# Hxyz-123/GoMatching

Hardware: AMD Instinct MI355X
Metric: frames/sec (whole node), 1280x720 clip, 100 queries/frame (higher is better)
Workload: dtype f32 (f16x3 split MFMA: 22-bit significand products, fp32 accumulate; parity tests at fp32 tolerances)

## Files before the change

### gomatching_amd/csrc/bneck_fused.hip

```cpp
#include "common.h"

namespace {

constexpr int CH = 32;
constexpr int FRAG = 1024;
constexpr int BM = 128;
constexpr int XT_ROW = 36;

struct BnArgs {
    const float* A;
    const unsigned char* img;
    const float* R;
    const float* sc1;
    const float* sh1;
    float* X;
    float* Y1;
    int* flag;
    int lda, ldr, ldx, ldy, M, chunks;
};

template <int K1, int MP>
struct Cfg {
    static constexpr int W3_FRAGS = (K1 / 16) * 2;
    static constexpr int W1_FRAGS = (MP / 32) * 2 * 2;
    static constexpr int STAGE_FRAGS = W3_FRAGS + W1_FRAGS + 1;
    static constexpr int STAGE_BYTES = STAGE_FRAGS * FRAG;
    static constexpr int XTR = (K1 == 64 && MP == 64) ? 32 : 16;
    static constexpr int XT_BYTES = XTR * XT_ROW * 4;
    static constexpr int LDS_BYTES = 2 * STAGE_BYTES + 4 * XT_BYTES;
};

template <int K1, int MP, int OCC>
__global__ __launch_bounds__(256, OCC) void bneck_kernel(const BnArgs p) {
    using C = Cfg<K1, MP>;
    extern __shared__ __attribute__((aligned(16))) unsigned char smem[];
    const int tid = threadIdx.x, lane = tid & 63;
    const int wave = __builtin_amdgcn_readfirstlane(tid >> 6);
    const int fr = lane & 31, fh = lane >> 5;
    const long m = (long)blockIdx.x * BM + wave * 32 + fr;
    const long row = m < p.M ? m : p.M - 1;
    const unsigned lane16 = lane * 16;

    const __amdgpu_buffer_rsrc_t rs_img = gom_buffer_rsrc(p.img, p.chunks * C::STAGE_BYTES);
    auto dma_stage = [&](int c, int slot) {
        for (int f = wave; f < C::STAGE_FRAGS; f += 4)
            gom_dma_fragment(rs_img, lane16, (unsigned)c * C::STAGE_BYTES + f * FRAG, smem + slot * C::STAGE_BYTES + f * FRAG);
    };

    float amax = 0.f, chk = 0.f;
    half8 xf[2][K1 / 16];
    long crow[4];
#pragma unroll
    for (int i = 0; i < 4; ++i) {
        const long mm = (long)blockIdx.x * BM + wave * 32 + (lane >> 3) + 8 * i;
        crow[i] = mm < p.M ? mm : p.M - 1;
    }
    const int cpc = (lane & 7) * 4;
    float* xt = reinterpret_cast<float*>(smem + 2 * C::STAGE_BYTES + wave * C::XT_BYTES);
    constexpr int XTR = C::XTR, PASSES = 32 / XTR, RPP = XTR / 8;
    f32x4 rv[4];
    {
        const float* xr = p.A + (size_t)row * p.lda + fh * 8;
        f32x4 ra[K1 / 8];
#pragma unroll
        for (int s = 0; s < K1 / 16; ++s) {
            ra[2 * s] = *reinterpret_cast<const f32x4*>(xr + 16 * s);
            ra[2 * s + 1] = *reinterpret_cast<const f32x4*>(xr + 16 * s + 4);
        }
#pragma unroll
        for (int i = 0; i < 4; ++i) rv[i] = *reinterpret_cast<const f32x4*>(p.R + (size_t)crow[i] * p.ldr + cpc);
        __builtin_amdgcn_sched_barrier(0);
        dma_stage(0, 0);
        __builtin_amdgcn_sched_barrier(0);
#pragma unroll
        for (int s = 0; s < K1 / 16; ++s) {
#pragma unroll
            for (int e = 0; e < 4; ++e) amax = fmaxf(amax, fmaxf(fabsf(ra[2 * s][e]), fabsf(ra[2 * s + 1][e])));
            gom_split8_f16(ra[2 * s], ra[2 * s + 1], xf[0][s], xf[1][s]);
        }
        asm volatile("" : "+v"(amax));
    }

    f32x16 acc2[MP / 32];
#pragma unroll
    for (int t = 0; t < MP / 32; ++t)
#pragma unroll
        for (int g = 0; g < 16; ++g) acc2[t][g] = 0.f;

    asm volatile("s_waitcnt vmcnt(0)" ::: "memory");
    __syncthreads();

    for (int c = 0; c < p.chunks; ++c) {
        const int st = c & 1;
        const unsigned char* base = smem + st * C::STAGE_BYTES + lane16;
        const float* aux = reinterpret_cast<const float*>(smem + st * C::STAGE_BYTES + (C::W3_FRAGS + C::W1_FRAGS) * FRAG);
        if (c + 1 < p.chunks) dma_stage(c + 1, st ^ 1);
        f32x4 rn[4];
#pragma unroll
        for (int q = 0; q < 4; ++q) {
            rn[q] = f32x4{0.f, 0.f, 0.f, 0.f};
            if (c + 1 < p.chunks) rn[q] = *reinterpret_cast<const f32x4*>(p.R + (size_t)crow[q] * p.ldr + CH * (c + 1) + cpc);
        }
        f32x4 ra4[4];
#pragma unroll
        for (int hp = 0; hp < PASSES; ++hp) {
#pragma unroll
            for (int i = 0; i < RPP; ++i) *reinterpret_cast<f32x4*>(xt + ((lane >> 3) + 8 * i) * XT_ROW + cpc) = rv[RPP * hp + i];
            __builtin_amdgcn_wave_barrier();
            if (PASSES == 1 || (fr >> 4) == hp) {
#pragma unroll
                for (int q = 0; q < 4; ++q) ra4[q] = *reinterpret_cast<const f32x4*>(xt + (fr & (XTR - 1)) * XT_ROW + 8 * q + 4 * fh);
            }
            __builtin_amdgcn_wave_barrier();
        }
        f32x16 acc1;
#pragma unroll
        for (int g = 0; g < 16; ++g) acc1[g] = 0.f;
#pragma unroll
        for (int s = 0; s < K1 / 16; ++s) {
            const half8 w_hi = *reinterpret_cast<const half8*>(base + (2 * s) * FRAG);
            const half8 w_lo = *reinterpret_cast<const half8*>(base + (2 * s + 1) * FRAG);
            acc1 = __builtin_amdgcn_mfma_f32_32x32x16_f16(w_hi, xf[1][s], acc1, 0, 0, 0);
            acc1 = __builtin_amdgcn_mfma_f32_32x32x16_f16(w_lo, xf[0][s], acc1, 0, 0, 0);
            acc1 = __builtin_amdgcn_mfma_f32_32x32x16_f16(w_hi, xf[0][s], acc1, 0, 0, 0);
        }
        half8 hf[2][2];
        f32x4 vx[4];
#pragma unroll
        for (int u = 0; u < 2; ++u) {
            f32x4 v[2];
#pragma unroll
            for (int qq = 0; qq < 2; ++qq) {
                const int q = 2 * u + qq;
                const f32x4 sc = *reinterpret_cast<const f32x4*>(aux + 8 * q + 4 * fh);
                const f32x4 sh = *reinterpret_cast<const f32x4*>(aux + CH + 8 * q + 4 * fh);
#pragma unroll
                for (int e = 0; e < 4; ++e) {
                    const float t = acc1[4 * q + e] * sc[e] + sh[e] + ra4[q][e];
                    chk = fmaf(t, 0.f, chk);
                    v[qq][e] = fmaxf(t, 0.f);
                    amax = fmaxf(amax, v[qq][e]);
                }
                vx[q] = v[qq];
            }
            gom_split8_f16(v[0], v[1], hf[0][u], hf[1][u]);
        }
#pragma unroll
        for (int hp = 0; hp < PASSES; ++hp) {
            if (PASSES == 1 || (fr >> 4) == hp) {
#pragma unroll
                for (int q = 0; q < 4; ++q) *reinterpret_cast<f32x4*>(xt + (fr & (XTR - 1)) * XT_ROW + 8 * q + 4 * fh) = vx[q];
            }
            __builtin_amdgcn_wave_barrier();
#pragma unroll
            for (int i = 0; i < RPP; ++i) {
                const f32x4 o = *reinterpret_cast<const f32x4*>(xt + ((lane >> 3) + 8 * i) * XT_ROW + cpc);
                *reinterpret_cast<f32x4*>(p.X + (size_t)crow[RPP * hp + i] * p.ldx + CH * c + cpc) = o;
            }
            __builtin_amdgcn_wave_barrier();
        }
#pragma unroll
        for (int t = 0; t < MP / 32; ++t)
#pragma unroll
            for (int u = 0; u < 2; ++u) {
                const half8 w_hi = *reinterpret_cast<const half8*>(base + (C::W3_FRAGS + (t * 2 + u) * 2) * FRAG);
                const half8 w_lo = *reinterpret_cast<const half8*>(base + (C::W3_FRAGS + (t * 2 + u) * 2 + 1) * FRAG);
                acc2[t] = __builtin_amdgcn_mfma_f32_32x32x16_f16(w_hi, hf[1][u], acc2[t], 0, 0, 0);
                acc2[t] = __builtin_amdgcn_mfma_f32_32x32x16_f16(w_lo, hf[0][u], acc2[t], 0, 0, 0);
                acc2[t] = __builtin_amdgcn_mfma_f32_32x32x16_f16(w_hi, hf[0][u], acc2[t], 0, 0, 0);
            }
#pragma unroll
        for (int q = 0; q < 4; ++q) rv[q] = rn[q];
        asm volatile("s_waitcnt vmcnt(4)" ::: "memory");
        __syncthreads();
    }

    float* yrow = p.Y1 + (size_t)row * p.ldy + 4 * fh;
#pragma unroll
    for (int t = 0; t < MP / 32; ++t)
#pragma unroll
        for (int q = 0; q < 4; ++q) {
            const int col = 32 * t + 8 * q + 4 * fh;
            const f32x4 sc = *reinterpret_cast<const f32x4*>(p.sc1 + col);
            const f32x4 sh = *reinterpret_cast<const f32x4*>(p.sh1 + col);
            f32x4 o;
#pragma unroll
            for (int e = 0; e < 4; ++e) {
                const float tv = acc2[t][4 * q + e] * sc[e] + sh[e];
                chk = fmaf(tv, 0.f, chk);
                o[e] = fmaxf(tv, 0.f);
            }
            *reinterpret_cast<f32x4*>(yrow + 32 * t + 8 * q) = o;
        }
    if ((!(amax <= 65504.f) || !(chk == 0.f)) && p.flag) atomicOr(p.flag, 1);
}

__global__ __launch_bounds__(256) void bneck_image_kernel(const unsigned short* __restrict__ p3, long ps3, int ld3,
                                                          const float* __restrict__ inv3, const float* __restrict__ scale3,
                                                          const float* __restrict__ shift3, const unsigned short* __restrict__ p1,
                                                          long ps1, int ld1, int k1, int c4, int mp, unsigned short* __restrict__ img) {
    const int w3f = (k1 / 16) * 2, w1f = (mp / 32) * 4, sf = w3f + w1f + 1;
    const long i = (long)blockIdx.x * 256 + threadIdx.x;
    const long total = (long)(c4 / CH) * sf * 512;
    if (i >= total) return;
    const int e = (int)(i % 512), f = (int)((i / 512) % sf), c = (int)(i / (512L * sf));
    const int l = e >> 3, j = e & 7, r = l & 31, h = l >> 5;
    if (f < w3f) {
        const int s = f >> 1, pl = f & 1;
        img[i] = p3[pl * ps3 + (size_t)(CH * c + r) * ld3 + 16 * s + 8 * h + j];
    } else if (f < w3f + w1f) {
        const int id = f - w3f, t = id >> 2, u = (id >> 1) & 1, pl = id & 1;
        img[i] = p1[pl * ps1 + (size_t)(32 * t + r) * ld1 + CH * c + 16 * u + 8 * (j >> 2) + 4 * h + (j & 3)];
    } else {
        const int fi = e >> 1;
        float v = 0.f;
        if (fi < CH) v = inv3[CH * c + fi] * (scale3 ? scale3[CH * c + fi] : 1.f);
        else if (fi < 2 * CH) v = shift3 ? shift3[CH * c + fi - CH] : 0.f;
        const unsigned bits = __builtin_bit_cast(unsigned, v);
        img[i] = (unsigned short)((e & 1) ? (bits >> 16) : (bits & 0xffffu));
    }
}

template <int K1, int MP, int OCC>
int launch(const BnArgs& a, hipStream_t s) {
    using C = Cfg<K1, MP>;
    auto kern = bneck_kernel<K1, MP, OCC>;
    if (C::LDS_BYTES > 65536) {
        hipError_t e = hipFuncSetAttribute((const void*)kern, hipFuncAttributeMaxDynamicSharedMemorySize, C::LDS_BYTES);
        if (e != hipSuccess) return GOM_ERR_HIP_BASE + (int)e;
    }
    hipLaunchKernelGGL(kern, dim3((unsigned)cdiv(a.M, BM)), dim3(256), C::LDS_BYTES, s, a);
    return gom_launch_status();
}

bool served(int k1, int c4, int mp) {
    if (c4 != 4 * k1) return false;
    return (k1 == 64 && (mp == 64 || mp == 128)) || (k1 == 128 && (mp == 128 || mp == 256));
}

}

extern "C" long gom_bneck_image_bytes(int k1, int c4, int mp) {
    if (!served(k1, c4, mp)) return -1;
    return (long)(c4 / CH) * ((k1 / 16) * 2 + (mp / 32) * 4 + 1) * FRAG;
}

extern "C" int gom_bneck_image(const void* w3_planes, long w3_plane_stride, int ld3, const float* w3_inv_scale, const float* scale3,
                               const float* shift3, const void* w1_planes, long w1_plane_stride, int ld1, int k1, int c4, int mp,
                               void* image, long image_bytes, void* stream) {
    GOM_CHECK_ARG(w3_planes && w3_inv_scale && w1_planes && image && served(k1, c4, mp) && ld3 >= k1 && ld1 >= c4);
    GOM_CHECK_ARG(image_bytes >= gom_bneck_image_bytes(k1, c4, mp));
    const long total = (long)(c4 / CH) * ((k1 / 16) * 2 + (mp / 32) * 4 + 1) * 512;
    hipLaunchKernelGGL(bneck_image_kernel, dim3((unsigned)cdiv(total, 256)), dim3(256), 0, (hipStream_t)stream,
                       (const unsigned short*)w3_planes, w3_plane_stride, ld3, w3_inv_scale, scale3, shift3,
                       (const unsigned short*)w1_planes, w1_plane_stride, ld1, k1, c4, mp, (unsigned short*)image);
    return gom_launch_status();
}

extern "C" int gom_bneck_f32(const float* A, int lda, const void* image, const float* R, int ldr, const float* scale1,
                             const float* shift1, float* X, int ldx, float* Y1, int ldy, int M, int k1, int c4, int mp, int* flag,
                             void* stream) {
    GOM_CHECK_ARG(A && image && R && scale1 && shift1 && X && Y1 && M >= 0 && served(k1, c4, mp));
    GOM_CHECK_ARG(lda >= k1 && ldr >= c4 && ldx >= c4 && ldy >= mp && (lda % 4) == 0 && (ldr % 4) == 0 && (ldx % 4) == 0 && (ldy % 4) == 0);
    GOM_CHECK_ARG(((uintptr_t)A % 16) == 0 && ((uintptr_t)R % 16) == 0 && ((uintptr_t)X % 16) == 0 && ((uintptr_t)Y1 % 16) == 0 &&
                  ((uintptr_t)image % 16) == 0 && ((uintptr_t)scale1 % 16) == 0 && ((uintptr_t)shift1 % 16) == 0);
    if (M == 0) return GOM_OK;
    BnArgs a{};
    a.A = A; a.img = (const unsigned char*)image; a.R = R; a.sc1 = scale1; a.sh1 = shift1; a.X = X; a.Y1 = Y1; a.flag = flag;
    a.lda = lda; a.ldr = ldr; a.ldx = ldx; a.ldy = ldy; a.M = M; a.chunks = c4 / CH;
    hipStream_t s = (hipStream_t)stream;
    if (k1 == 64 && mp == 64) return launch<64, 64, 3>(a, s);
    if (k1 == 64 && mp == 128) return launch<64, 128, 2>(a, s);
    if (k1 == 128 && mp == 128) return launch<128, 128, 2>(a, s);
    return launch<128, 256, 1>(a, s);
}
```

### gomatching_amd/lib.py

```python
import ctypes
import os
from ctypes import c_int, c_long, c_float, c_void_p

HERE = os.path.dirname(os.path.abspath(__file__))
LIB_PATH = os.environ.get("GOM_LIB_PATH") or os.path.join(HERE, "libgomatching_hip.so")

GOM_OK = 0
_ERR = {1: "GOM_ERR_INVALID_ARG (violated precondition)", 2: "GOM_ERR_UNSUPPORTED"}

P = c_void_p
I = c_int
L = c_long
F = c_float

SIGNATURES = {
    "gom_abi_version": (I, []),
    "gom_built_for_arch": (ctypes.c_char_p, []),
    "gom_ms_deform_attn_forward": (I, [P, P, P, P, P, P, I, I, I, I, I, I, I, P]),
    "gom_ms_deform_attn_forward_any": (I, [I, P, P, P, P, P, P, I, I, I, I, I, I, I, P]),
    "gom_ms_deform_attn_backward": (I, [I, P, P, P, P, P, P, P, P, P, I, I, I, I, I, I, I, P]),
    "gom_ms_deform_attn_forward_strided": (I, [P, L, I, P, P, P, P, P, I, I, P]),
    "gom_msda_set_lane_distributed": (I, [I]),
    "gom_msda_fused_forward": (I, [P, I, P, P, L, I, P, P, P, I, I, P]),
    "gom_msda_fused_forward_encoder": (I, [P, I, P, P, L, I, P, P, P, I, I, I, I, I, I, P]),
    "gom_msda_set_window": (I, [I]),
    "gom_msda_window_count_fallbacks": (I, [P]),
    "gom_msda_prepare": (I, [P, I, P, I, P, P, P, L, P]),
    "gom_gemm_f32": (I, [P, P, P, I, P, I, P, P, P, I, I, P, I, I, I, I, P]),
    "gom_gemm_splitk_workspace_bytes": (L, [I, I, I]),
    "gom_gemm_f32_splitk": (I, [P, P, I, P, I, P, P, P, I, I, P, I, I, I, I, P, L, P]),
    "gom_conv2d_nhwc_f32": (I, [P, P, P, P, P, I, P, I, I, I, I, I, I, I, I, I, P]),
    "gom_split_bf16x3": (I, [P, I, I, I, P, I, P]),
    "gom_gemm_f32_bf16x6": (I, [P, P, I, P, L, I, P, P, P, I, I, I, P, I, I, I, I, P]),
    "gom_conv2d_nhwc_f32_bf16x6": (I, [P, P, L, I, P, P, P, I, P, I, I, I, I, I, I, I, I, I, P]),
    "gom_gemm_small_f32": (I, [P, P, I, P, I, P, P, P, I, I, P, I, I, I, I, P]),
    "gom_conv_bf16x6_splits": (I, [I, I, I]),
    "gom_conv2d_nhwc_f32_bf16x6_splitk": (I, [P, P, L, I, P, P, P, I, P, I, I, I, I, I, I, I, I, I, P, L, I, P]),
    "gom_split_f16x2": (I, [P, I, I, I, P, I, P, P]),
    "gom_gemm_f32_f16x3": (I, [P, P, I, P, L, I, P, P, P, P, I, I, I, P, I, I, I, I, P, P]),
    "gom_gemm_f32_f16x3_rp": (I, [P, P, I, P, L, I, P, P, P, P, I, I, I, I, P, I, I, I, I, P, P]),
    "gom_conv2d_nhwc_f32_f16x3": (I, [P, P, L, I, P, P, P, P, I, P, I, I, I, I, I, I, I, I, I, P, L, I, P, P]),
    "gom_conv3x3_patch_supported": (I, [I, I]),
    "gom_conv3x3_patch_image_bytes": (L, [I, I]),
    "gom_conv3x3_patch_image": (I, [P, L, I, I, I, P, L, P]),
    "gom_conv3x3_patch_f32_f16x3": (I, [P, P, P, P, P, I, P, I, I, I, I, I, P, P]),
    "gom_bneck_image_bytes": (L, [I, I, I]),
    "gom_bneck_image": (I, [P, L, I, P, P, P, P, L, I, I, I, I, P, L, P]),
    "gom_bneck_f32": (I, [P, I, P, P, I, P, P, P, I, P, I, I, I, I, I, P, P]),
    "gom_bneck2_image_bytes": (L, [I, I, I]),
    "gom_bneck2_image": (I, [P, L, I, P, P, P, P, L, I, I, I, I, P, L, P]),
    "gom_bneck2_f32": (I, [P, I, P, P, I, P, P, P, I, P, I, I, I, I, I, P, P]),
    "gom_dec_attn_image_bytes": (L, [I, I]),
    "gom_dec_attn_image": (I, [P, L, I, P, P, P, L, I, P, P, P, P, I, P, L, P]),
    "gom_dec_attn_f32": (I, [P, I, P, I, P, F, P, I, I, I, I, I, P, P]),
    "gom_dec_attn_raw_image_bytes": (L, []),
    "gom_dec_attn_raw_image": (I, [P, L, I, P, P, P, L, P]),
    "gom_dec_attn_raw_f32": (I, [P, I, P, F, P, I, P, I, P, I, I, I, I, P, P]),
    "gom_dec_attn2_image_bytes": (L, [I, I]),
    "gom_dec_attn2_image": (I, [P, L, I, P, P, P, L, I, P, P, P, P, I, P, L, P]),
    "gom_dec_attn2_f32": (I, [P, I, P, I, P, F, P, I, I, I, I, I, P, P]),
    "gom_dec_attn2_raw_image_bytes": (L, []),
    "gom_dec_attn2_raw_image": (I, [P, L, I, P, P, P, L, P]),
    "gom_dec_attn2_raw_f32": (I, [P, I, P, F, P, I, P, I, P, I, I, I, I, P, P]),
    "gom_dec_inter_heads_f32": (I, [P, I, P, P, I, I, I, I, P, P]),
    "gom_proj_ln_image_bytes": (L, [I, I]),
    "gom_proj_ln_image": (I, [P, L, I, I, I, P, L, P]),
    "gom_proj_ln_f32": (I, [P, I, P, P, P, P, I, P, P, F, P, I, I, P, P]),
    "gom_proj_ln_dot_f32": (I, [P, I, P, P, P, P, P, F, P, F, P, I, P, P]),
    "gom_gemm_k256_image_bytes": (L, [I, I]),
    "gom_gemm_k256_image": (I, [P, L, I, P, P, I, I, P, L, P]),
    "gom_gemm_k256_f32": (I, [P, P, I, P, P, I, I, I, P, I, I, I, I, I, P, P]),
    "gom_gemm_k256_rp_f32": (I, [P, P, I, P, P, I, I, I, I, P, I, I, I, I, I, P, P]),
    "gom_gemm_k256_set_lines": (None, [I]),
    "gom_gemm_k256_set_interleave": (None, [I]),
    "gom_stem_conv_pool_f32": (I, [P, P, L, I, P, P, P, P, I, I, I, P, P]),
    "gom_ffn_fused_image_bytes": (L, [I, I]),
    "gom_ffn_fused_image": (I, [P, L, I, P, P, P, L, I, I, I, P, L, P]),
    "gom_ffn_set_half_tail": (I, [I]),
    "gom_ffn_set_stream_cus": (I, [I]),
    "gom_ffn_fused_ln_f32": (I, [P, I, P, P, P, P, P, F, P, I, I, I, I, P, P]),
    "gom_ffn_fused_image_acc_order": (I, [P, L, I, P, P, P, L, I, I, I, P, L, P]),
# ... 114 lines not shown
```

### gomatching_amd/modeling/backbone.py

```python
import torch

from .. import ops

_STAGES = (("res2", 3, 1), ("res3", 4, 2), ("res4", 6, 2), ("res5", 3, 2))


def _fold_bn(sd, name, device, eps=1e-5):
    scale = sd[name + ".norm.weight"] * (sd[name + ".norm.running_var"] + eps).rsqrt()
    shift = sd[name + ".norm.bias"] - sd[name + ".norm.running_mean"] * scale
    return scale.float().contiguous().to(device), shift.float().contiguous().to(device)


def _ohwi(w, device, pad_cin_to=None):
    w = w.float().permute(0, 2, 3, 1)
    if pad_cin_to is not None and w.shape[-1] < pad_cin_to:
        w = torch.cat([w, w.new_zeros(w.shape[:-1] + (pad_cin_to - w.shape[-1],))], -1)
    return w.contiguous().to(device)


class ResNet50:
    out_features = ("res3", "res4", "res5")
    strides = {"res3": 8, "res4": 16, "res5": 32}
    channels = {"res3": 512, "res4": 1024, "res5": 2048}

    def __init__(self, sd, device, prefix="backbone.0.backbone."):
        self.device = device
        self.convs = {}

        def add(name, pad_cin_to=None):
            w = ops.prep_conv_weight(_ohwi(sd[prefix + name + ".weight"], device, pad_cin_to))
            sc, sh = _fold_bn(sd, prefix + name, device)
            self.convs[name] = (w, sc, sh)

        add("stem.conv1", pad_cin_to=4)
        self.blocks = []
        for stage, nblk, first_stride in _STAGES:
            for i in range(nblk):
                p = "%s.%d." % (stage, i)
                has_sc = (prefix + p + "shortcut.weight") in sd
                if has_sc:
                    add(p + "shortcut")
                for c in ("conv1", "conv2", "conv3"):
                    add(p + c)
                self.blocks.append((stage, p, first_stride if i == 0 else 1, has_sc, i == nblk - 1))
        self.fused = {}
        for (_, p, _, _, _), (_, pn, _, _, _) in zip(self.blocks[:-1], self.blocks[1:]):
            w3, sc3, sh3 = self.convs[p + "conv3"]
            w1, sc1, sh1 = self.convs[pn + "conv1"]
            if ops.BneckFused.serves(w3, w1):
                self.fused[p] = ops.BneckFused(w3, sc3, sh3, w1, sc1, sh1)

    def _conv(self, x, name, stride=1, pad=0, relu=False, R=None):
        w, sc, sh = self.convs[name]
        return ops.conv2d_nhwc(x, w, scale=sc, shift=sh, R=R, relu=relu, stride=stride, pad=pad)

    def forward(self, x_nhwc4):
        w, sc, sh = self.convs["stem.conv1"]
        if ops.stem_pool_serves(w):
            x = ops.stem_conv_pool(x_nhwc4.contiguous(), w, scale=sc, shift=sh)
        else:
            x = self._conv(x_nhwc4, "stem.conv1", stride=2, pad=3, relu=True)
            x = ops.maxpool3x3s2(x)
        outs = {}
        y1 = None
        for stage, p, s, has_sc, last in self.blocks:
            sc = self._conv(x, p + "shortcut", stride=s) if has_sc else x
            y = y1 if y1 is not None else self._conv(x, p + "conv1", relu=True)
            y = self._conv(y, p + "conv2", stride=s, pad=1, relu=True)
            blk = self.fused.get(p)
            if blk is not None:
                x, y1 = ops.bneck_fused(y, blk, sc)
            else:
                x, y1 = self._conv(y, p + "conv3", relu=True, R=sc), None
            if last:
                outs[stage] = x
        return {k: outs[k] for k in self.out_features}
```

### gomatching_amd/ops.py

```python
import contextlib
import ctypes
import math

import numpy as np
import torch

from . import lib as _lib_mod
from .lib import check

_f32 = torch.float32


def _L():
    return _lib_mod.load()


_gemm_profile = None


_profile_scope = ""


@contextlib.contextmanager
def profile_scope(name):
# ... 503 lines not shown
    if prof is not None:
        e1.record()
        prof.append((e0, e1, 2.0 * M * 256 * 256, (12.0 if R is not None else 8.0) * M * 256 + blk.image.numel(),
                     "projln:%dx256x256" % M, _profile_scope))
    return out


PROPOSAL_DOT = _switch("PROPOSAL_DOT")


def proj_ln_dot(x, blk, w, b):
    assert x.dim() == 2 and x.stride(1) == 1 and x.shape[1] == 256 and x.dtype == _f32
    _chk_f32(w)
    assert w.numel() == 256
    M = x.shape[0]
    out = torch.empty((M,), dtype=_f32, device=x.device)
    prof = _gemm_profile if (_gemm_profile is not None and M > 0) else None
    if prof is not None:
        e0, e1 = torch.cuda.Event(enable_timing=True), torch.cuda.Event(enable_timing=True)
        e0.record()
    check(_L().gom_proj_ln_dot_f32(_p(x), x.stride(0) if M > 1 else 256, _p(blk.image), _p(blk.W.inv_scale), _p(blk.bias),
                                   _p(blk.gamma), _p(blk.beta), blk.eps, _p(w), float(b), _p(out), M, _p(range_flag(x.device)),
                                   _stream()), "gom_proj_ln_dot_f32")
    if prof is not None:
        e1.record()
        prof.append((e0, e1, 2.0 * M * 256 * 257, 4.0 * M * 257 + blk.image.numel(), "projdot:%dx256x257" % M, _profile_scope))
    return out


BNECK_FUSED = _switch("BNECK_FUSED")


BNECK2 = _switch("BNECK2")


class BneckFused:

    def __init__(self, w3, scale3, shift3, w1, scale1, shift1):
        assert isinstance(w3, SplitWeight) and isinstance(w1, SplitWeight) and w3.kind == "f16x3" and w1.kind == "f16x3"
        self.k1, self.c4, self.mp = w3.K, w3.N, w1.N
        assert w1.K == self.c4
        _chk_f32(scale3, shift3, scale1, shift1)
        p3, p1 = w3.planes, w1.planes
        self.v2 = BneckFused._wide(self.k1, self.c4, self.mp)
        if self.v2:
            nbytes = _L().gom_bneck2_image_bytes(self.k1, self.c4, self.mp)
            self.image = torch.empty((nbytes,), dtype=torch.uint8, device=p3.device)
            check(_L().gom_bneck2_image(_p(p3), p3.stride(0), p3.stride(1), _p(w3.inv_scale), _p(scale3), _p(shift3), _p(p1), p1.stride(0),
                                        p1.stride(1), self.k1, self.c4, self.mp, _p(self.image), nbytes, _stream()), "gom_bneck2_image")
            self.sc1 = (scale1 * w1.inv_scale).contiguous()
            self.sh1 = shift1.contiguous()
            return
        nbytes = _L().gom_bneck_image_bytes(self.k1, self.c4, self.mp)
        if nbytes < 0:
            raise _lib_mod.GomError("fused bottleneck kernel does not serve %d -> %d -> %d" % (self.k1, self.c4, self.mp))
        self.image = torch.empty((nbytes,), dtype=torch.uint8, device=p3.device)
        check(_L().gom_bneck_image(_p(p3), p3.stride(0), p3.stride(1), _p(w3.inv_scale), _p(scale3), _p(shift3), _p(p1), p1.stride(0),
                                   p1.stride(1), self.k1, self.c4, self.mp, _p(self.image), nbytes, _stream()), "gom_bneck_image")
        self.sc1 = (scale1 * w1.inv_scale).contiguous()
        self.sh1 = shift1.contiguous()

    @staticmethod
    def _wide(k1, c4, mp):
        return bool(BNECK2) and _L().gom_bneck2_image_bytes(k1, c4, mp) > 0

    @staticmethod
    def serves(w3, w1):
        return (BNECK_FUSED and GEMM_MODE == "f16x3" and isinstance(w3, SplitWeight) and isinstance(w1, SplitWeight)
                and w3.kind == "f16x3" and w1.kind == "f16x3" and w1.K == w3.N
                and (BneckFused._wide(w3.K, w3.N, w1.N) or _L().gom_bneck_image_bytes(w3.K, w3.N, w1.N) > 0))


def bneck_fused(a, blk, R):
    _chk_f32(a, R)
    B, H, W, k1 = a.shape
    assert k1 == blk.k1 and tuple(R.shape) == (B, H, W, blk.c4) and a.is_contiguous() and R.is_contiguous()
    M = B * H * W
    X = torch.empty((B, H, W, blk.c4), dtype=_f32, device=a.device)
    Y1 = torch.empty((B, H, W, blk.mp), dtype=_f32, device=a.device)
    prof = _gemm_profile if (_gemm_profile is not None and M > 0) else None
    if prof is not None:
        e0, e1 = torch.cuda.Event(enable_timing=True), torch.cuda.Event(enable_timing=True)
        e0.record()
    fn = _L().gom_bneck2_f32 if blk.v2 else _L().gom_bneck_f32
    check(fn(_p(a), k1, _p(blk.image), _p(R), blk.c4, _p(blk.sc1), _p(blk.sh1), _p(X), blk.c4, _p(Y1), blk.mp, M,
             blk.k1, blk.c4, blk.mp, _p(range_flag(a.device)), _stream()), "gom_bneck2_f32" if blk.v2 else "gom_bneck_f32")
    if prof is not None:
        e1.record()
        prof.append((e0, e1, 2.0 * M * blk.c4 * (blk.k1 + blk.mp), 4.0 * M * (blk.k1 + 2 * blk.c4 + blk.mp) + blk.image.numel(),
                     "bneck:%dx%dx%dx%d" % (M, blk.k1, blk.c4, blk.mp), _profile_scope))
    return X, Y1


DEC_ATTN = _switch("DEC_ATTN")
DEC_ATTN_INTRA = _switch("DEC_ATTN_INTRA")
DEC_ATTN_INTER = _switch("DEC_ATTN_INTER")


class DecAttnBlock:

    def __init__(self, in_w, in_b, out_w, out_b, gamma, beta, inter, eps=1e-5, raw=None, form=None):
        self.form = form if form is not None else (2 if DEC_ATTN2 else 1)
        assert tuple(in_w.shape) == (768, 256) and tuple(out_w.shape) == (256, 256)
        nbytes = _L().gom_dec_attn_image_bytes(256, 8)
        if nbytes < 0:
            raise _lib_mod.GomError("decoder attention kernel serves d_model 256 / 8 heads only")
# ... 1071 lines not shown
```

### include/gomatching_hip.h

```cpp
#ifndef GOMATCHING_HIP_H_
#define GOMATCHING_HIP_H_

#include <stdint.h>

#ifdef __cplusplus
extern "C" {
#endif

#define GOM_OK 0
#define GOM_ERR_INVALID_ARG 1
#define GOM_ERR_UNSUPPORTED 2
#define GOM_ERR_HIP_BASE 1000

#define GOM_DTYPE_F32 0
#define GOM_DTYPE_F64 1

#define GOM_ABI_VERSION 1
int gom_abi_version(void);
const char* gom_built_for_arch(void);

int gom_ms_deform_attn_forward(const float* value, const int64_t* spatial_shapes, const int64_t* level_start_index,
                               const float* sampling_loc, const float* attn_weight, float* output, int batch,
                               int spatial_size, int num_heads, int channels, int num_levels, int num_query,
                               int num_point, void* stream);
// ... 58 lines not shown
                       int relu, float* C, int ldc, int M, int N, int K, int* flag, void* stream);
int gom_gemm_f32_f16x3_rp(const float* A, const int* a_rows, int lda, const void* Wplanes, long w_plane_stride, int ldw,
                          const float* wscale, const float* scale, const float* shift, const float* R, int ldr, int r_cols,
                          int r_period, int relu, float* C, int ldc, int M, int N, int K, int* flag, void* stream);
int gom_conv2d_nhwc_f32_f16x3(const float* X, const void* Wplanes, long w_plane_stride, int ldw, const float* wscale,
                              const float* scale, const float* shift, const float* R, int relu, float* Y, int B, int H,
                              int Wd, int Cin, int Cout, int KH, int KW, int stride, int pad, void* workspace,
                              long workspace_bytes, int splits, int* flag, void* stream);
int gom_conv3x3_patch_supported(int Cin, int Cout);
long gom_conv3x3_patch_image_bytes(int Cin, int Cout);
int gom_conv3x3_patch_image(const void* w_planes, long w_plane_stride, int ldw, int Cin, int Cout, void* image, long image_bytes,
                            void* stream);
int gom_conv3x3_patch_f32_f16x3(const float* X, const void* image, const float* wscale, const float* scale, const float* shift,
                                int relu, float* Y, int B, int H, int Wd, int Cin, int Cout, int* flag, void* stream);
int gom_stem_conv_pool_f32(const float* X, const void* Wplanes, long w_plane_stride, int ldw, const float* wscale,
                           const float* scale, const float* shift, float* Y, int B, int H, int Wd, int* flag, void* stream);

long gom_proj_ln_image_bytes(int n, int k);
int gom_proj_ln_image(const void* w_planes, long w_plane_stride, int ldw, int n, int k, void* image, long image_bytes,
                      void* stream);
int gom_proj_ln_f32(const float* X, int ldx, const void* image, const float* w_inv_scale, const float* bias, const float* R,
                    int ldr, const float* gamma, const float* beta, float eps, float* Y, int ldy, int M, int* flag,
                    void* stream);
int gom_proj_ln_dot_f32(const float* X, int ldx, const void* image, const float* w_inv_scale, const float* bias,
                        const float* gamma, const float* beta, float eps, const float* dot_w, float dot_b, float* out, int M,
                        int* flag, void* stream);

long gom_bneck_image_bytes(int k1, int c4, int mp);
int gom_bneck_image(const void* w3_planes, long w3_plane_stride, int ld3, const float* w3_inv_scale, const float* scale3,
                    const float* shift3, const void* w1_planes, long w1_plane_stride, int ld1, int k1, int c4, int mp, void* image,
                    long image_bytes, void* stream);
int gom_bneck_f32(const float* A, int lda, const void* image, const float* R, int ldr, const float* scale1, const float* shift1,
                  float* X, int ldx, float* Y1, int ldy, int M, int k1, int c4, int mp, int* flag, void* stream);
long gom_bneck2_image_bytes(int k1, int c4, int mp);
int gom_bneck2_image(const void* w3_planes, long w3_plane_stride, int ld3, const float* w3_inv_scale, const float* scale3,
                     const float* shift3, const void* w1_planes, long w1_plane_stride, int ld1, int k1, int c4, int mp, void* image,
                     long image_bytes, void* stream);
int gom_bneck2_f32(const float* A, int lda, const void* image, const float* R, int ldr, const float* scale1, const float* shift1,
                   float* X, int ldx, float* Y1, int ldy, int M, int k1, int c4, int mp, int* flag, void* stream);

long gom_dec_attn_image_bytes(int d_model, int heads);
int gom_dec_attn_image(const void* in_planes, long in_plane_stride, int ld_in, const float* in_inv_scale, const float* in_bias,
                       const void* out_planes, long out_plane_stride, int ld_out, const float* out_inv_scale,
                       const float* out_bias, const float* gamma, const float* beta, int inter, void* image, long image_bytes,
                       void* stream);
int gom_dec_attn_f32(const float* X, int ldx, const float* P, int ldp, const void* image, float eps, float* Y, int ldy, int groups,
                     int group_tokens, int inner, int inter, int* flag, void* stream);
long gom_dec_attn_raw_image_bytes(void);
int gom_dec_attn_raw_image(const void* raw_planes, long raw_plane_stride, int ld_raw, const float* raw_inv_scale,
                           const float* raw_bias, void* image, long image_bytes, void* stream);
int gom_dec_attn_raw_f32(const float* X, int ldx, const void* image, float eps, float* Y, int ldy, const float* P2, int ldp2,
                         float* raw, int ldraw, int groups, int group_tokens, int inner, int* flag, void* stream);

long gom_dec_attn2_image_bytes(int d_model, int heads);
int gom_dec_attn2_image(const void* in_planes, long in_plane_stride, int ld_in, const float* in_inv_scale, const float* in_bias,
                        const void* out_planes, long out_plane_stride, int ld_out, const float* out_inv_scale,
                        const float* out_bias, const float* gamma, const float* beta, int inter, void* image, long image_bytes,
                        void* stream);
int gom_dec_attn2_f32(const float* X, int ldx, const float* P, int ldp, const void* image, float eps, float* Y, int ldy, int groups,
                      int group_tokens, int inner, int inter, int* flag, void* stream);
long gom_dec_attn2_raw_image_bytes(void);
int gom_dec_attn2_raw_image(const void* raw_planes, long raw_plane_stride, int ld_raw, const float* raw_inv_scale,
                            const float* raw_bias, void* image, long image_bytes, void* stream);
int gom_dec_attn2_raw_f32(const float* X, int ldx, const void* image, float eps, float* Y, int ldy, const float* P2, int ldp2,
                          float* raw, int ldraw, int groups, int group_tokens, int inner, int* flag, void* stream);

// ... 231 lines not shown
```

Before: 307.3.

## Fuse projection shortcut conv into fused bottleneck conv3+conv1 kernel

Adds a shortcut variant of the fused bottleneck kernel that computes the 1x1 projection shortcut conv (with its BN scale/shift) in-register via f16x3 MFMAs instead of reading a precomputed residual tensor. The shortcut weights and scale/shift are packed into the per-chunk weight image, and the residual-transpose path is skipped. This removes a separate shortcut conv launch and the write and read of its c4-wide output. In exchange each chunk does extra MFMAs, the LDS stage grows, and it is served only for k1=64, c4=256, mp=64, stride 1, behind a BNECK_SHORTCUT switch.

Result: faster. 311.2 (median of 6 runs) (+1.3%).

```diff
diff --git a/gomatching_amd/csrc/bneck_fused.hip b/gomatching_amd/csrc/bneck_fused.hip
--- a/gomatching_amd/csrc/bneck_fused.hip
+++ b/gomatching_amd/csrc/bneck_fused.hip
@@ -17,22 +17,26 @@
     float* Y1;
     int* flag;
     int lda, ldr, ldx, ldy, M, chunks;
+    const float* S;
+    int lds, Hs, Ws, OH, OW;
 };
 
-template <int K1, int MP>
+template <int K1, int MP, int KS>
 struct Cfg {
     static constexpr int W3_FRAGS = (K1 / 16) * 2;
     static constexpr int W1_FRAGS = (MP / 32) * 2 * 2;
-    static constexpr int STAGE_FRAGS = W3_FRAGS + W1_FRAGS + 1;
+    static constexpr int WS_FRAGS = (KS / 16) * 2;
+    static constexpr int STAGE_FRAGS = W3_FRAGS + W1_FRAGS + 1 + WS_FRAGS;
     static constexpr int STAGE_BYTES = STAGE_FRAGS * FRAG;
     static constexpr int XTR = (K1 == 64 && MP == 64) ? 32 : 16;
     static constexpr int XT_BYTES = XTR * XT_ROW * 4;
     static constexpr int LDS_BYTES = 2 * STAGE_BYTES + 4 * XT_BYTES;
 };
 
-template <int K1, int MP, int OCC>
+template <int K1, int MP, int OCC, int KS, int STRIDE>
 __global__ __launch_bounds__(256, OCC) void bneck_kernel(const BnArgs p) {
-    using C = Cfg<K1, MP>;
+    using C = Cfg<K1, MP, KS>;
+    constexpr bool SC = KS > 0;
     extern __shared__ __attribute__((aligned(16))) unsigned char smem[];
     const int tid = threadIdx.x, lane = tid & 63;
     const int wave = __builtin_amdgcn_readfirstlane(tid >> 6);
@@ -59,6 +63,7 @@
     float* xt = reinterpret_cast<float*>(smem + 2 * C::STAGE_BYTES + wave * C::XT_BYTES);
     constexpr int XTR = C::XTR, PASSES = 32 / XTR, RPP = XTR / 8;
     f32x4 rv[4];
+    half8 sf[2][SC ? KS / 16 : 1];
     {
         const float* xr = p.A + (size_t)row * p.lda + fh * 8;
         f32x4 ra[K1 / 8];
@@ -67,8 +72,25 @@
             ra[2 * s] = *reinterpret_cast<const f32x4*>(xr + 16 * s);
             ra[2 * s + 1] = *reinterpret_cast<const f32x4*>(xr + 16 * s + 4);
         }
-#pragma unroll
-        for (int i = 0; i < 4; ++i) rv[i] = *reinterpret_cast<const f32x4*>(p.R + (size_t)crow[i] * p.ldr + cpc);
+        f32x4 rs[SC ? KS / 8 : 1];
+        if constexpr (SC) {
+            long srow = row;
+            if constexpr (STRIDE != 1) {
+                const int ohw = p.OH * p.OW;
+                const int b = (int)(row / ohw), rem = (int)(row - (long)b * ohw);
+                const int y = rem / p.OW, x = rem - y * p.OW;
+                srow = ((long)b * p.Hs + STRIDE * y) * p.Ws + STRIDE * x;
+            }
+            const float* sr = p.S + (size_t)srow * p.lds + fh * 8;
+#pragma unroll
+            for (int s = 0; s < KS / 16; ++s) {
+                rs[2 * s] = *reinterpret_cast<const f32x4*>(sr + 16 * s);
+                rs[2 * s + 1] = *reinterpret_cast<const f32x4*>(sr + 16 * s + 4);
+            }
+        } else {
+#pragma unroll
+            for (int i = 0; i < 4; ++i) rv[i] = *reinterpret_cast<const f32x4*>(p.R + (size_t)crow[i] * p.ldr + cpc);
+        }
         __builtin_amdgcn_sched_barrier(0);
         dma_stage(0, 0);
         __builtin_amdgcn_sched_barrier(0);
@@ -77,6 +99,14 @@
 #pragma unroll
             for (int e = 0; e < 4; ++e) amax = fmaxf(amax, fmaxf(fabsf(ra[2 * s][e]), fabsf(ra[2 * s + 1][e])));
             gom_split8_f16(ra[2 * s], ra[2 * s + 1], xf[0][s], xf[1][s]);
+        }
+        if constexpr (SC) {
+#pragma unroll
+            for (int s = 0; s < KS / 16; ++s) {
+#pragma unroll
+                for (int e = 0; e < 4; ++e) amax = fmaxf(amax, fmaxf(fabsf(rs[2 * s][e]), fabsf(rs[2 * s + 1][e])));
+                gom_split8_f16(rs[2 * s], rs[2 * s + 1], sf[0][s], sf[1][s]);
+            }
         }
         asm volatile("" : "+v"(amax));
     }
@@ -96,14 +126,16 @@
         const float* aux = reinterpret_cast<const float*>(smem + st * C::STAGE_BYTES + (C::W3_FRAGS + C::W1_FRAGS) * FRAG);
         if (c + 1 < p.chunks) dma_stage(c + 1, st ^ 1);
         f32x4 rn[4];
-#pragma unroll
-        for (int q = 0; q < 4; ++q) {
-            rn[q] = f32x4{0.f, 0.f, 0.f, 0.f};
-            if (c + 1 < p.chunks) rn[q] = *reinterpret_cast<const f32x4*>(p.R + (size_t)crow[q] * p.ldr + CH * (c + 1) + cpc);
+        if constexpr (!SC) {
+#pragma unroll
+            for (int q = 0; q < 4; ++q) {
+                rn[q] = f32x4{0.f, 0.f, 0.f, 0.f};
+                if (c + 1 < p.chunks) rn[q] = *reinterpret_cast<const f32x4*>(p.R + (size_t)crow[q] * p.ldr + CH * (c + 1) + cpc);
+            }
         }
         f32x4 ra4[4];
 #pragma unroll
-        for (int hp = 0; hp < PASSES; ++hp) {
+        for (int hp = 0; hp < (SC ? 0 : PASSES); ++hp) {
 #pragma unroll
             for (int i = 0; i < RPP; ++i) *reinterpret_cast<f32x4*>(xt + ((lane >> 3) + 8 * i) * XT_ROW + cpc) = rv[RPP * hp + i];
             __builtin_amdgcn_wave_barrier();
@@ -124,6 +156,19 @@
             acc1 = __builtin_amdgcn_mfma_f32_32x32x16_f16(w_lo, xf[0][s], acc1, 0, 0, 0);
             acc1 = __builtin_amdgcn_mfma_f32_32x32x16_f16(w_hi, xf[0][s], acc1, 0, 0, 0);
         }
+        f32x16 accs;
+        if constexpr (SC) {
+#pragma unroll
+            for (int g = 0; g < 16; ++g) accs[g] = 0.f;
+#pragma unroll
+            for (int s = 0; s < KS / 16; ++s) {
+                const half8 w_hi = *reinterpret_cast<const half8*>(base + (C::W3_FRAGS + C::W1_FRAGS + 1 + 2 * s) * FRAG);
+                const half8 w_lo = *reinterpret_cast<const half8*>(base + (C::W3_FRAGS + C::W1_FRAGS + 1 + 2 * s + 1) * FRAG);
+                accs = __builtin_amdgcn_mfma_f32_32x32x16_f16(w_hi, sf[1][s], accs, 0, 0, 0);
+                accs = __builtin_amdgcn_mfma_f32_32x32x16_f16(w_lo, sf[0][s], accs, 0, 0, 0);
+                accs = __builtin_amdgcn_mfma_f32_32x32x16_f16(w_hi, sf[0][s], accs, 0, 0, 0);
+            }
+        }
         half8 hf[2][2];
         f32x4 vx[4];
 #pragma unroll
@@ -134,6 +179,12 @@
                 const int q = 2 * u + qq;
                 const f32x4 sc = *reinterpret_cast<const f32x4*>(aux + 8 * q + 4 * fh);
                 const f32x4 sh = *reinterpret_cast<const f32x4*>(aux + CH + 8 * q + 4 * fh);
+                if constexpr (SC) {
+                    const f32x4 scs = *reinterpret_cast<const f32x4*>(aux + 2 * CH + 8 * q + 4 * fh);
+                    const f32x4 shs = *reinterpret_cast<const f32x4*>(aux + 3 * CH + 8 * q + 4 * fh);
+#pragma unroll
+                    for (int e = 0; e < 4; ++e) ra4[q][e] = accs[4 * q + e] * scs[e] + shs[e];
+                }
 #pragma unroll
                 for (int e = 0; e < 4; ++e) {
                     const float t = acc1[4 * q + e] * sc[e] + sh[e] + ra4[q][e];
@@ -169,8 +220,10 @@
                 acc2[t] = __builtin_amdgcn_mfma_f32_32x32x16_f16(w_lo, hf[0][u], acc2[t], 0, 0, 0);
                 acc2[t] = __builtin_amdgcn_mfma_f32_32x32x16_f16(w_hi, hf[0][u], acc2[t], 0, 0, 0);
             }
-#pragma unroll
-        for (int q = 0; q < 4; ++q) rv[q] = rn[q];
+        if constexpr (!SC) {
+#pragma unroll
+            for (int q = 0; q < 4; ++q) rv[q] = rn[q];
+        }
         asm volatile("s_waitcnt vmcnt(4)" ::: "memory");
         __syncthreads();
     }
@@ -195,11 +248,19 @@
     if ((!(amax <= 65504.f) || !(chk == 0.f)) && p.flag) atomicOr(p.flag, 1);
 }
 
+struct ImgSc {
+    const unsigned short* p;
+    long ps;
+    int ld, ks;
+    const float *inv, *scale, *shift;
+};
+
 __global__ __launch_bounds__(256) void bneck_image_kernel(const unsigned short* __restrict__ p3, long ps3, int ld3,
                                                           const float* __restrict__ inv3, const float* __restrict__ scale3,
                                                           const float* __restrict__ shift3, const unsigned short* __restrict__ p1,
-                                                          long ps1, int ld1, int k1, int c4, int mp, unsigned short* __restrict__ img) {
-    const int w3f = (k1 / 16) * 2, w1f = (mp / 32) * 4, sf = w3f + w1f + 1;
+                                                          long ps1, int ld1, int k1, int c4, int mp, const ImgSc sc,
+                                                          unsigned short* __restrict__ img) {
+    const int w3f = (k1 / 16) * 2, w1f = (mp / 32) * 4, sf = w3f + w1f + 1 + (sc.ks / 16) * 2;
     const long i = (long)blockIdx.x * 256 + threadIdx.x;
     const long total = (long)(c4 / CH) * sf * 512;
     if (i >= total) return;
@@ -211,20 +272,25 @@
     } else if (f < w3f + w1f) {
         const int id = f - w3f, t = id >> 2, u = (id >> 1) & 1, pl = id & 1;
         img[i] = p1[pl * ps1 + (size_t)(32 * t + r) * ld1 + CH * c + 16 * u + 8 * (j >> 2) + 4 * h + (j & 3)];
-    } else {
+    } else if (f == w3f + w1f) {
         const int fi = e >> 1;
         float v = 0.f;
         if (fi < CH) v = inv3[CH * c + fi] * (scale3 ? scale3[CH * c + fi] : 1.f);
         else if (fi < 2 * CH) v = shift3 ? shift3[CH * c + fi - CH] : 0.f;
+        else if (sc.ks > 0 && fi < 3 * CH) v = sc.inv[CH * c + fi - 2 * CH] * (sc.scale ? sc.scale[CH * c + fi - 2 * CH] : 1.f);
+        else if (sc.ks > 0 && fi < 4 * CH) v = sc.shift ? sc.shift[CH * c + fi - 3 * CH] : 0.f;
         const unsigned bits = __builtin_bit_cast(unsigned, v);
         img[i] = (unsigned short)((e & 1) ? (bits >> 16) : (bits & 0xffffu));
-    }
-}
-
-template <int K1, int MP, int OCC>
+    } else {
+        const int id = f - (w3f + w1f + 1), s = id >> 1, pl = id & 1;
+        img[i] = sc.p[pl * sc.ps + (size_t)(CH * c + r) * sc.ld + 16 * s + 8 * h + j];
+    }
+}
+
+template <int K1, int MP, int OCC, int KS = 0, int STRIDE = 1>
 int launch(const BnArgs& a, hipStream_t s) {
-    using C = Cfg<K1, MP>;
-    auto kern = bneck_kernel<K1, MP, OCC>;
+    using C = Cfg<K1, MP, KS>;
+    auto kern = bneck_kernel<K1, MP, OCC, KS, STRIDE>;
     if (C::LDS_BYTES > 65536) {
         hipError_t e = hipFuncSetAttribute((const void*)kern, hipFuncAttributeMaxDynamicSharedMemorySize, C::LDS_BYTES);
         if (e != hipSuccess) return GOM_ERR_HIP_BASE + (int)e;
@@ -238,11 +304,29 @@
     return (k1 == 64 && (mp == 64 || mp == 128)) || (k1 == 128 && (mp == 128 || mp == 256));
 }
 
+bool served_sc(int k1, int c4, int mp, int ks, int stride) {
+    return k1 == 64 && c4 == 256 && mp == 64 && ks == 64 && stride == 1;
+}
+
+long image_bytes(int k1, int c4, int mp, int ks) {
+    return (long)(c4 / CH) * ((k1 / 16) * 2 + (mp / 32) * 4 + 1 + (ks / 16) * 2) * FRAG;
+}
+
+int make_image(const void* w3_planes, long w3_plane_stride, int ld3, const float* w3_inv_scale, const float* scale3,
+               const float* shift3, const void* w1_planes, long w1_plane_stride, int ld1, int k1, int c4, int mp, const ImgSc& sc,
+               void* image, void* stream) {
+    const long total = image_bytes(k1, c4, mp, sc.ks) / 2;
+    hipLaunchKernelGGL(bneck_image_kernel, dim3((unsigned)cdiv(total, 256)), dim3(256), 0, (hipStream_t)stream,
+                       (const unsigned short*)w3_planes, w3_plane_stride, ld3, w3_inv_scale, scale3, shift3,
+                       (const unsigned short*)w1_planes, w1_plane_stride, ld1, k1, c4, mp, sc, (unsigned short*)image);
+    return gom_launch_status();
+}
+
 }
 
 extern "C" long gom_bneck_image_bytes(int k1, int c4, int mp) {
     if (!served(k1, c4, mp)) return -1;
-    return (long)(c4 / CH) * ((k1 / 16) * 2 + (mp / 32) * 4 + 1) * FRAG;
+    return image_bytes(k1, c4, mp, 0);
 }
 
 extern "C" int gom_bneck_image(const void* w3_planes, long w3_plane_stride, int ld3, const float* w3_inv_scale, const float* scale3,
@@ -250,11 +334,8 @@
                                void* image, long image_bytes, void* stream) {
     GOM_CHECK_ARG(w3_planes && w3_inv_scale && w1_planes && image && served(k1, c4, mp) && ld3 >= k1 && ld1 >= c4);
     GOM_CHECK_ARG(image_bytes >= gom_bneck_image_bytes(k1, c4, mp));
-    const long total = (long)(c4 / CH) * ((k1 / 16) * 2 + (mp / 32) * 4 + 1) * 512;
-    hipLaunchKernelGGL(bneck_image_kernel, dim3((unsigned)cdiv(total, 256)), dim3(256), 0, (hipStream_t)stream,
-                       (const unsigned short*)w3_planes, w3_plane_stride, ld3, w3_inv_scale, scale3, shift3,
-                       (const unsigned short*)w1_planes, w1_plane_stride, ld1, k1, c4, mp, (unsigned short*)image);
-    return gom_launch_status();
+    return make_image(w3_planes, w3_plane_stride, ld3, w3_inv_scale, scale3, shift3, w1_planes, w1_plane_stride, ld1, k1, c4, mp,
+                      ImgSc{}, image, stream);
 }
 
 extern "C" int gom_bneck_f32(const float* A, int lda, const void* image, const float* R, int ldr, const float* scale1,
@@ -274,3 +355,38 @@
     if (k1 == 128 && mp == 128) return launch<128, 128, 2>(a, s);
     return launch<128, 256, 1>(a, s);
 }
+
+extern "C" long gom_bneck_sc_image_bytes(int k1, int c4, int mp, int ks, int stride) {
+    if (!served_sc(k1, c4, mp, ks, stride)) return -1;
+    return image_bytes(k1, c4, mp, ks);
+}
+
+extern "C" int gom_bneck_sc_image(const void* w3_planes, long w3_plane_stride, int ld3, const float* w3_inv_scale, const float* scale3,
+                                  const float* shift3, const void* w1_planes, long w1_plane_stride, int ld1,
+                                  const void* ws_planes, long ws_plane_stride, int lds, const float* ws_inv_scale, const float* scale_s,
+                                  const float* shift_s, int k1, int c4, int mp, int ks, int stride, void* image, long image_bytes,
+                                  void* stream) {
+    GOM_CHECK_ARG(w3_planes && w3_inv_scale && w1_planes && ws_planes && ws_inv_scale && image && served_sc(k1, c4, mp, ks, stride));
+    GOM_CHECK_ARG(ld3 >= k1 && ld1 >= c4 && lds >= ks && image_bytes >= gom_bneck_sc_image_bytes(k1, c4, mp, ks, stride));
+    const ImgSc sc{(const unsigned short*)ws_planes, ws_plane_stride, lds, ks, ws_inv_scale, scale_s, shift_s};
+    return make_image(w3_planes, w3_plane_stride, ld3, w3_inv_scale, scale3, shift3, w1_planes, w1_plane_stride, ld1, k1, c4, mp, sc,
+                      image, stream);
+}
+
+extern "C" int gom_bneck_sc_f32(const float* A, int lda, const void* image, const float* S, int lds, int B, int Hs, int Ws, int stride,
+                                const float* scale1, const float* shift1, float* X, int ldx, float* Y1, int ldy, int k1, int c4, int mp,
+                                int ks, int* flag, void* stream) {
+    GOM_CHECK_ARG(A && image && S && scale1 && shift1 && X && Y1 && B >= 0 && Hs > 0 && Ws > 0 && served_sc(k1, c4, mp, ks, stride));
+    GOM_CHECK_ARG(lda >= k1 && lds >= ks && ldx >= c4 && ldy >= mp && (lda % 4) == 0 && (lds % 4) == 0 && (ldx % 4) == 0 && (ldy % 4) == 0);
+    GOM_CHECK_ARG(((uintptr_t)A % 16) == 0 && ((uintptr_t)S % 16) == 0 && ((uintptr_t)X % 16) == 0 && ((uintptr_t)Y1 % 16) == 0 &&
+                  ((uintptr_t)image % 16) == 0 && ((uintptr_t)scale1 % 16) == 0 && ((uintptr_t)shift1 % 16) == 0);
+    const int OH = (Hs - 1) / stride + 1, OW = (Ws - 1) / stride + 1;
+    const long M = (long)B * OH * OW;
+    GOM_CHECK_ARG(M <= 0x7fffffffL);
+    if (M == 0) return GOM_OK;
+    BnArgs a{};
+    a.A = A; a.img = (const unsigned char*)image; a.S = S; a.sc1 = scale1; a.sh1 = shift1; a.X = X; a.Y1 = Y1; a.flag = flag;
+    a.lda = lda; a.lds = lds; a.ldx = ldx; a.ldy = ldy; a.M = (int)M; a.chunks = c4 / CH;
+    a.Hs = Hs; a.Ws = Ws; a.OH = OH; a.OW = OW;
+    return launch<64, 64, 2, 64, 1>(a, (hipStream_t)stream);
+}
diff --git a/gomatching_amd/lib.py b/gomatching_amd/lib.py
--- a/gomatching_amd/lib.py
+++ b/gomatching_amd/lib.py
@@ -47,6 +47,9 @@
     "gom_bneck_image_bytes": (L, [I, I, I]),
     "gom_bneck_image": (I, [P, L, I, P, P, P, P, L, I, I, I, I, P, L, P]),
     "gom_bneck_f32": (I, [P, I, P, P, I, P, P, P, I, P, I, I, I, I, I, P, P]),
+    "gom_bneck_sc_image_bytes": (L, [I, I, I, I, I]),
+    "gom_bneck_sc_image": (I, [P, L, I, P, P, P, P, L, I, P, L, I, P, P, P, I, I, I, I, I, P, L, P]),
+    "gom_bneck_sc_f32": (I, [P, I, P, P, I, I, I, I, I, P, P, P, I, P, I, I, I, I, I, P, P]),
     "gom_bneck2_image_bytes": (L, [I, I, I]),
     "gom_bneck2_image": (I, [P, L, I, P, P, P, P, L, I, I, I, I, P, L, P]),
     "gom_bneck2_f32": (I, [P, I, P, P, I, P, P, P, I, P, I, I, I, I, I, P, P]),
diff --git a/gomatching_amd/modeling/backbone.py b/gomatching_amd/modeling/backbone.py
--- a/gomatching_amd/modeling/backbone.py
+++ b/gomatching_amd/modeling/backbone.py
@@ -44,11 +44,14 @@
                     add(p + c)
                 self.blocks.append((stage, p, first_stride if i == 0 else 1, has_sc, i == nblk - 1))
         self.fused = {}
-        for (_, p, _, _, _), (_, pn, _, _, _) in zip(self.blocks[:-1], self.blocks[1:]):
+        for (_, p, s, has_sc, _), (_, pn, _, _, _) in zip(self.blocks[:-1], self.blocks[1:]):
             w3, sc3, sh3 = self.convs[p + "conv3"]
             w1, sc1, sh1 = self.convs[pn + "conv1"]
             if ops.BneckFused.serves(w3, w1):
-                self.fused[p] = ops.BneckFused(w3, sc3, sh3, w1, sc1, sh1)
+                shortcut = None
+                if has_sc and ops.BneckFused.serves_shortcut(w3, w1, self.convs[p + "shortcut"][0], s):
+                    shortcut = self.convs[p + "shortcut"] + (s,)
+                self.fused[p] = ops.BneckFused(w3, sc3, sh3, w1, sc1, sh1, shortcut=shortcut)
 
     def _conv(self, x, name, stride=1, pad=0, relu=False, R=None):
         w, sc, sh = self.convs[name]
@@ -64,10 +67,13 @@
         outs = {}
         y1 = None
         for stage, p, s, has_sc, last in self.blocks:
-            sc = self._conv(x, p + "shortcut", stride=s) if has_sc else x
+            blk = self.fused.get(p)
+            if blk is not None and blk.ks:
+                sc = x
+            else:
+                sc = self._conv(x, p + "shortcut", stride=s) if has_sc else x
             y = y1 if y1 is not None else self._conv(x, p + "conv1", relu=True)
             y = self._conv(y, p + "conv2", stride=s, pad=1, relu=True)
-            blk = self.fused.get(p)
             if blk is not None:
                 x, y1 = ops.bneck_fused(y, blk, sc)
             else:
diff --git a/gomatching_amd/ops.py b/gomatching_amd/ops.py
--- a/gomatching_amd/ops.py
+++ b/gomatching_amd/ops.py
@@ -559,16 +559,33 @@
 
 
 BNECK2 = _switch("BNECK2")
+BNECK_SHORTCUT = _switch("BNECK_SHORTCUT")
 
 
 class BneckFused:
 
-    def __init__(self, w3, scale3, shift3, w1, scale1, shift1):
+    def __init__(self, w3, scale3, shift3, w1, scale1, shift1, shortcut=None):
         assert isinstance(w3, SplitWeight) and isinstance(w1, SplitWeight) and w3.kind == "f16x3" and w1.kind == "f16x3"
         self.k1, self.c4, self.mp = w3.K, w3.N, w1.N
         assert w1.K == self.c4
         _chk_f32(scale3, shift3, scale1, shift1)
         p3, p1 = w3.planes, w1.planes
+        self.ks, self.stride = 0, 1
+        if shortcut is not None:
+            ws, scale_s, shift_s, stride = shortcut
+            assert BneckFused.serves_shortcut(w3, w1, ws, stride), "fused bottleneck kernel does not serve this shortcut"
+            _chk_f32(scale_s, shift_s)
+            self.v2, self.ks, self.stride = False, ws.K, int(stride)
+            ps = ws.planes
+            nbytes = _L().gom_bneck_sc_image_bytes(self.k1, self.c4, self.mp, self.ks, self.stride)
+            self.image = torch.empty((nbytes,), dtype=torch.uint8, device=p3.device)
+            check(_L().gom_bneck_sc_image(_p(p3), p3.stride(0), p3.stride(1), _p(w3.inv_scale), _p(scale3), _p(shift3), _p(p1),
+                                          p1.stride(0), p1.stride(1), _p(ps), ps.stride(0), ps.stride(1), _p(ws.inv_scale),
+                                          _p(scale_s), _p(shift_s), self.k1, self.c4, self.mp, self.ks, self.stride, _p(self.image),
+                                          nbytes, _stream()), "gom_bneck_sc_image")
+            self.sc1 = (scale1 * w1.inv_scale).contiguous()
+            self.sh1 = shift1.contiguous()
+            return
         self.v2 = BneckFused._wide(self.k1, self.c4, self.mp)
         if self.v2:
             nbytes = _L().gom_bneck2_image_bytes(self.k1, self.c4, self.mp)
@@ -598,7 +615,38 @@
                 and (BneckFused._wide(w3.K, w3.N, w1.N) or _L().gom_bneck_image_bytes(w3.K, w3.N, w1.N) > 0))
 
 
+    @staticmethod
+    def serves_shortcut(w3, w1, ws, stride):
+        return (bool(BNECK_SHORTCUT) and BneckFused.serves(w3, w1) and isinstance(ws, SplitWeight) and ws.kind == "f16x3"
+                and ws.N == w3.N and _L().gom_bneck_sc_image_bytes(w3.K, w3.N, w1.N, ws.K, int(stride)) > 0)
+
+
+def _bneck_fused_sc(a, blk, S):
+    _chk_f32(a, S)
+    B, H, W, k1 = a.shape
+    Bs, Hs, Ws, ks = S.shape
+    st = blk.stride
+    assert k1 == blk.k1 and ks == blk.ks and Bs == B and (H, W) == ((Hs - 1) // st + 1, (Ws - 1) // st + 1)
+    assert a.is_contiguous() and S.is_contiguous()
+    M = B * H * W
+    X = torch.empty((B, H, W, blk.c4), dtype=_f32, device=a.device)
+    Y1 = torch.empty((B, H, W, blk.mp), dtype=_f32, device=a.device)
+    prof = _gemm_profile if (_gemm_profile is not None and M > 0) else None
+    if prof is not None:
+        e0, e1 = torch.cuda.Event(enable_timing=True), torch.cuda.Event(enable_timing=True)
+        e0.record()
+    check(_L().gom_bneck_sc_f32(_p(a), k1, _p(blk.image), _p(S), ks, B, Hs, Ws, st, _p(blk.sc1), _p(blk.sh1), _p(X), blk.c4, _p(Y1),
+                                blk.mp, blk.k1, blk.c4, blk.mp, blk.ks, _p(range_flag(a.device)), _stream()), "gom_bneck_sc_f32")
+    if prof is not None:
+        e1.record()
+        prof.append((e0, e1, 2.0 * M * blk.c4 * (blk.k1 + blk.ks + blk.mp), 4.0 * M * (blk.k1 + blk.ks + blk.c4 + blk.mp) + blk.image.numel(),
+                     "bneck:%dx%dx%dx%d+sc%d/%d" % (M, blk.k1, blk.c4, blk.mp, blk.ks, st), _profile_scope))
+    return X, Y1
+
+
 def bneck_fused(a, blk, R):
+    if blk.ks:
+        return _bneck_fused_sc(a, blk, R)
     _chk_f32(a, R)
     B, H, W, k1 = a.shape
     assert k1 == blk.k1 and tuple(R.shape) == (B, H, W, blk.c4) and a.is_contiguous() and R.is_contiguous()
diff --git a/include/gomatching_hip.h b/include/gomatching_hip.h
--- a/include/gomatching_hip.h
+++ b/include/gomatching_hip.h
@@ -114,6 +114,14 @@
                     long image_bytes, void* stream);
 int gom_bneck_f32(const float* A, int lda, const void* image, const float* R, int ldr, const float* scale1, const float* shift1,
                   float* X, int ldx, float* Y1, int ldy, int M, int k1, int c4, int mp, int* flag, void* stream);
+long gom_bneck_sc_image_bytes(int k1, int c4, int mp, int ks, int stride);
+int gom_bneck_sc_image(const void* w3_planes, long w3_plane_stride, int ld3, const float* w3_inv_scale, const float* scale3,
+                       const float* shift3, const void* w1_planes, long w1_plane_stride, int ld1, const void* ws_planes,
+                       long ws_plane_stride, int lds, const float* ws_inv_scale, const float* scale_s, const float* shift_s, int k1,
+                       int c4, int mp, int ks, int stride, void* image, long image_bytes, void* stream);
+int gom_bneck_sc_f32(const float* A, int lda, const void* image, const float* S, int lds, int B, int Hs, int Ws, int stride,
+                     const float* scale1, const float* shift1, float* X, int ldx, float* Y1, int ldy, int k1, int c4, int mp, int ks,
+                     int* flag, void* stream);
 long gom_bneck2_image_bytes(int k1, int c4, int mp);
 int gom_bneck2_image(const void* w3_planes, long w3_plane_stride, int ld3, const float* w3_inv_scale, const float* scale3,
                      const float* shift3, const void* w1_planes, long w1_plane_stride, int ld1, int k1, int c4, int mp, void* image,
```
